# jgrss/cultionet

Measured on AMD Instinct MI355X. Metric: train_chips_per_sec, higher is better.
Workload: dtype f32

## Files before the change

### cultionet_amd/csrc/cn_conv.hip

```cpp
#include "cn_common.h"
#include "cn_conv_geom.h"
#include "cn_profile.h"

#include <cstdlib>

#define KC 8

static int cn_reduce_slices(const CnConvGeom& g, hipStream_t stream);

template <int TN, int TM>
__device__ __forceinline__ void cn_igemm_epilogue(const CnConvGeom& g, const f32x16 (&acc)[TN][TM],
                                                  const bool (&pix_ok)[TM], const int (&out_off)[TM], int co_base,
                                                  int half, int grp, int split, int b,
                                                  const float* __restrict__ bias, float* __restrict__ y) {
  const int HWout = g.Hout * g.Wout;
  const bool sliced = g.slice_stride != 0;
  float* yb = sliced ? g.part + (long)(grp * g.splits + split) * g.slice_stride + (long)b * g.Cout * HWout
                     : y + (long)b * g.ybs;
  const bool first = split == 0;
#pragma unroll
  for (int tn = 0; tn < TN; ++tn) {
#pragma unroll
    for (int r = 0; r < 16; ++r) {
      const int co = co_base + tn * 32 + (r & 3) + 8 * (r >> 2) + 4 * half;
      if (co < g.Cout) {
        const float bv = (bias != nullptr && first) ? bias[co] : 0.f;
#pragma unroll
        for (int tm = 0; tm < TM; ++tm) {
          if (pix_ok[tm]) {
            float* dst = yb + (long)co * HWout + out_off[tm];
            const float v = acc[tn][tm][r] + bv;
            if (sliced) {
              *dst = acc[tn][tm][r];
            } else if (g.atomic_out) {
              atomicAdd(dst, v);
            } else if (g.accumulate) {
              *dst += v;
            } else {
              *dst = v;
            }
          }
        }
      }
    }
  }
}

template <int WAVES_N, int TN, int NI_T>
__global__ __launch_bounds__(256) void cn_conv_igemm_kernel(const CnConvGeom g) {
  constexpr int WAVES_M = 4 / WAVES_N;
  constexpr int MT = WAVES_M * 64;
  constexpr int NT = WAVES_N * TN * 32;
  constexpr int WI = (CN_MAX_TAPS * KC * (NT / 4) + 255) / 256;
  extern __shared__ __attribute__((aligned(16))) float smem[];
  float* in_lds = smem;
  float* w_lds = smem + g.w_lds_off;
  int* tap_lds = reinterpret_cast<int*>(smem + g.tap_lds_off);

  const int tid = threadIdx.x, lane = tid & 63, wid = tid >> 6;
  const int half = lane >> 5, l31 = lane & 31;
  const int wm = wid / WAVES_N, wn = wid % WAVES_N;

  int bx, by, split;
  if (!cn_xcd_block(g.grid_x, g.grid_y, g.grid_x * g.grid_y * g.splits, bx, by, split)) return;
  int ci_ = 0;
  if (g.interleave) {
    ci_ = bx % g.ncls;
  } else {
#pragma unroll 1
    for (int c = 1; c < g.ncls; ++c)
      if (bx >= g.cls[c].block_begin) ci_ = c;
  }
  const int grp = g.cls[ci_].grp;
  const float* __restrict__ x = g.gx[grp];
  const float* __restrict__ wp = g.gwp[grp];
  const float* __restrict__ bias = g.gbias[grp];
  float* __restrict__ y = g.gy[grp];
  const int Hg = g.cls[ci_].Hg, Wg = g.cls[ci_].Wg, ntaps = g.cls[ci_].ntaps;
  const int pitch = g.cls[ci_].pitch, plane = g.cls[ci_].plane;
  const int min_dy = g.cls[ci_].min_dy, min_dx = g.cls[ci_].min_dx;
  const int oy0 = g.cls[ci_].oy0, ox0 = g.cls[ci_].ox0;
  const int tiles_per_img = g.cls[ci_].tiles_per_img;
  const int tile = g.interleave ? bx / g.ncls : bx - g.cls[ci_].block_begin;
  const int b = tile / tiles_per_img;
  const int m0 = (tile - b * tiles_per_img) * MT;
  if (tid < ntaps) {
    tap_lds[tid] = (g.cls[ci_].dy[tid] - min_dy) * pitch + (g.cls[ci_].dx[tid] - min_dx);
    tap_lds[CN_MAX_TAPS + tid] = g.cls[ci_].wt[tid];
  }
  __syncthreads();
  const int n0 = by * NT;
  const int Mimg = Hg * Wg;
  const int gy0 = m0 / Wg;
  const int iy_base = gy0 * g.is + min_dy;
  const int HWin = g.Hin * g.Win;

  int goff[NI_T];
#pragma unroll
  for (int i = 0; i < NI_T; ++i) {
    const int e = tid + i * 256;
    if (e < plane) {
      const int r = e / pitch, c = e - r * pitch;
      const int iy = iy_base + r, ix = c + min_dx;
      goff[i] = (iy >= 0 && iy < g.Hin && ix >= 0 && ix < g.Win) ? iy * g.Win + ix : -1;
    } else {
      goff[i] = -2;
    }
  }

  int pix_lds[2], out_off[2];
  bool pix_ok[2];
#pragma unroll
  for (int tm = 0; tm < 2; ++tm) {
    const int p = m0 + wm * 64 + tm * 32 + l31;
    pix_ok[tm] = p < Mimg;
    const int pc = pix_ok[tm] ? p : Mimg - 1;
    const int gy = pc / Wg, gx = pc - gy * Wg;
    pix_lds[tm] = ((gy - gy0) * g.is) * pitch + gx * g.is + half * plane;
    out_off[tm] = (gy * g.os + oy0) * g.Wout + gx * g.os + ox0;
  }

  f32x16 acc[TN][2];
#pragma unroll
  for (int tn = 0; tn < TN; ++tn)
#pragma unroll
    for (int tm = 0; tm < 2; ++tm)
#pragma unroll
      for (int r = 0; r < 16; ++r) acc[tn][tm][r] = 0.f;

  const float* xb = x + (long)b * g.xbs;
  const int nw4 = ntaps * KC * (NT / 4);
  const int nchunks = (g.Cin + KC - 1) / KC;
  int ch = split * g.chunks_per_split;
  int ch_end = ch + g.chunks_per_split;
  if (ch_end > nchunks) ch_end = nchunks;

  if (ntaps > 0 && ch < ch_end) {
    float xin[KC][NI_T];
    f32x4 win[WI];
    constexpr unsigned CN_OOBD = 0x80000000u;
    const __amdgpu_buffer_rsrc_t xrs =
        __builtin_amdgcn_make_buffer_rsrc(const_cast<float*>(xb), 0, 0x7fffffff, 0x00020000);
    const __amdgpu_buffer_rsrc_t wrs =
        __builtin_amdgcn_make_buffer_rsrc(const_cast<float*>(wp), 0, 0x7fffffff, 0x00020000);
    unsigned xo[NI_T], wo[WI];
#pragma unroll
    for (int i = 0; i < NI_T; ++i) xo[i] = goff[i] >= 0 ? (unsigned)goff[i] * 4u : CN_OOBD;
#pragma unroll
    for (int j = 0; j < WI; ++j) {
      const int f = tid + j * 256;
      wo[j] = CN_OOBD;
      if (f < nw4) {
        const int row = f / (NT / 4), c4 = f - row * (NT / 4);
        const int t = row / KC, ci = row - t * KC;
        wo[j] = (unsigned)(((tap_lds[CN_MAX_TAPS + t] * g.Kpad + ci) * g.Npad + n0 + c4 * 4) * 4);
      }
    }
#define CN_PREFETCH(c0_)                                                                                   \
  {                                                                                                        \
    const int c0 = (c0_);                                                                                  \
    _Pragma("unroll") for (int ci = 0; ci < KC; ++ci) {                                                    \
      if ((c0 + ci) < g.Cin) {                                                           \
        const int so = (c0 + ci) * HWin * 4;                                                               \
        _Pragma("unroll") for (int i = 0; i < NI_T; ++i)                                                   \
            xin[ci][i] = __builtin_bit_cast(float, __builtin_amdgcn_raw_buffer_load_b32(xrs, xo[i], so, 0)); \
      } else {                                                                                             \
        _Pragma("unroll") for (int i = 0; i < NI_T; ++i) xin[ci][i] = 0.f;                                 \
      }                                                                                                    \
    }                                                                                                      \
    const int wso = c0 * g.Npad * 4;                                                                       \
    _Pragma("unroll") for (int j = 0; j < WI; ++j)                                                         \
        win[j] = __builtin_bit_cast(f32x4, __builtin_amdgcn_raw_buffer_load_b128(wrs, wo[j], wso, 0));     \
  }
    CN_PREFETCH(ch * KC);
    for (; ch < ch_end; ++ch) {
      __syncthreads();
#pragma unroll
      for (int ci = 0; ci < KC; ++ci)
#pragma unroll
        for (int i = 0; i < NI_T; ++i)
          if (goff[i] != -2) in_lds[ci * plane + tid + i * 256] = xin[ci][i];
#pragma unroll
      for (int j = 0; j < WI; ++j) {
        const int f = tid + j * 256;
        if (f < nw4) *reinterpret_cast<f32x4*>(w_lds + f * 4) = win[j];
      }
      __syncthreads();
      if (ch + 1 < ch_end) CN_PREFETCH((ch + 1) * KC);
      float opa[2][TN], opb[2][2];
#define CN_LOAD_OPS(bf_, t_, cp_, toff_)                                                                   \
  {                                                                                                        \
    const float* wrow = w_lds + ((t_) * KC + half) * NT + wn * (TN * 32) + l31;                            \
    _Pragma("unroll") for (int tn = 0; tn < TN; ++tn) opa[bf_][tn] = wrow[(2 * (cp_)) * NT + tn * 32];     \
    opb[bf_][0] = in_lds[pix_lds[0] + (2 * (cp_)) * plane + (toff_)];                                      \
    opb[bf_][1] = in_lds[pix_lds[1] + (2 * (cp_)) * plane + (toff_)];                                      \
  }
#define CN_MFMA(bf_)                                                                                       \
  _Pragma("unroll") for (int tn = 0; tn < TN; ++tn) _Pragma("unroll") for (int tm = 0; tm < 2; ++tm)       \
      acc[tn][tm] = __builtin_amdgcn_mfma_f32_32x32x2f32(opa[bf_][tn], opb[bf_][tm], acc[tn][tm], 0, 0, 0);
      int toff_cur = tap_lds[0];
      CN_LOAD_OPS(0, 0, 0, toff_cur);
#pragma unroll 1
      for (int t = 0; t < ntaps; ++t) {
        const int toff_nxt = (t + 1 < ntaps) ? tap_lds[t + 1] : 0;
        CN_LOAD_OPS(1, t, 1, toff_cur);
        CN_MFMA(0);
        CN_LOAD_OPS(0, t, 2, toff_cur);
        CN_MFMA(1);
        CN_LOAD_OPS(1, t, 3, toff_cur);
        CN_MFMA(0);
        if (t + 1 < ntaps) CN_LOAD_OPS(0, t + 1, 0, toff_nxt);
        CN_MFMA(1);
        toff_cur = toff_nxt;
      }
#undef CN_LOAD_OPS
#undef CN_MFMA
    }
#undef CN_PREFETCH
  }

  cn_igemm_epilogue<TN, 2>(g, acc, pix_ok, out_off, n0 + wn * (TN * 32), half, grp, split, b, bias, y);
}

template <int WAVES_N, int TN, int TM, int NV, int RP>
__global__ __launch_bounds__(256, (NV <= 1 ? 2 : 1)) void cn_conv_igemm_vec_kernel(const CnConvGeom g) {
  constexpr int WAVES_M = 4 / WAVES_N;
  constexpr int MT = WAVES_M * TM * 32;
  constexpr int NT = WAVES_N * TN * 32;
  constexpr int WI = (CN_MAX_TAPS * KC * (NT / 4) + 255) / 256;
  constexpr int VS = NV * 1024;
  constexpr bool PADR = RP == 1 || RP == 2;
  constexpr int ODD = RP == 3 ? 1 : 0;
  constexpr int VSS = VS + ODD;
  extern __shared__ __attribute__((aligned(16))) float smem[];
  float* in_lds = smem;
  float* w_lds = smem + g.w_lds_off;
  int* tap_lds = reinterpret_cast<int*>(smem + g.tap_lds_off);

  const int tid = threadIdx.x, lane = tid & 63, wid = tid >> 6;
  const int half = lane >> 5, l31 = lane & 31;
  const int wm = wid / WAVES_N, wn = wid % WAVES_N;

  int bx, by, split;
  if (!cn_xcd_block(g.grid_x, g.grid_y, g.grid_x * g.grid_y * g.splits, bx, by, split)) return;
  int ci_ = 0;
  if (g.interleave) {
    ci_ = bx % g.ncls;
  } else {
#pragma unroll 1
    for (int c = 1; c < g.ncls; ++c)
      if (bx >= g.cls[c].block_begin) ci_ = c;
  }
  const int grp = g.cls[ci_].grp;
  const float* __restrict__ x = g.gx[grp];
  const float* __restrict__ wp = g.gwp[grp];
  const float* __restrict__ bias = g.gbias[grp];
  float* __restrict__ y = g.gy[grp];
  const int Hg = g.cls[ci_].Hg, Wg = g.cls[ci_].Wg, ntaps = g.cls[ci_].ntaps;
  const int vplane = g.cls[ci_].vplane;
  const int min_dy = g.cls[ci_].min_dy, min_dx = g.cls[ci_].min_dx;
  const int oy0 = g.cls[ci_].oy0, ox0 = g.cls[ci_].ox0;
  const int tiles_per_img = g.cls[ci_].tiles_per_img;
  const int tile = g.interleave ? bx / g.ncls : bx - g.cls[ci_].block_begin;
  const int b = tile / tiles_per_img;
  const int m0 = (tile - b * tiles_per_img) * MT;
  const int Win = g.Win;
  const int pitch = PADR ? ((Win + 3) / 4 * 4 + 4) : Win;
  if (tid < ntaps) {
    tap_lds[tid] = PADR ? (g.cls[ci_].dy[tid] - min_dy) * pitch + g.cls[ci_].dx[tid]
                      : (g.cls[ci_].dy[tid] - min_dy) * Win + (g.cls[ci_].dx[tid] - min_dx);
    tap_lds[CN_MAX_TAPS + tid] = g.cls[ci_].wt[tid];
    tap_lds[2 * CN_MAX_TAPS + tid] = g.cls[ci_].dx[tid];
  }
  __syncthreads();
  const int n0 = by * NT;
  const int Mimg = Hg * Wg;
  const int gy0 = m0 / Wg;
  const int HWin = g.Hin * Win;
  const int start = PADR ? (gy0 * g.is + min_dy) * Win : (gy0 * g.is + min_dy) * Win + min_dx;
  const int f0 = (start >> 2) << 2;
  const int sh = start - f0;

  int goff[NV];
  int ldst[NV];
  int ldst2[NV];
#pragma unroll
  for (int i = 0; i < NV; ++i) {
    const int e4 = 4 * (tid + i * 256) - (PADR ? sh : 0);
    const int lim = PADR ? g.cls[ci_].rows * Win : vplane;
    ldst[i] = 0;
    ldst2[i] = 0;
    if (e4 + 3 >= 0 && e4 < lim) {
      const int fq = start + e4 - (PADR ? 0 : sh);
      goff[i] = (fq >= 0 && (ODD ? fq < HWin : fq + 3 < HWin)) ? fq : -1;
      if (RP == 1) {
        const int r = e4 / Win;
        ldst[i] = r * pitch + 4 + (e4 - r * Win);
      } else if (RP == 2) {
        const int ea = e4 < 0 ? e4 + 2 : e4, eb = e4 + 2;
        const int ra = ea / Win, rb = eb / Win;
        ldst[i] = e4 < 0 ? -1 : ra * pitch + 4 + (ea - ra * Win);
        ldst2[i] = eb < lim ? rb * pitch + 4 + (eb - rb * Win) : -1;
      } else {
        ldst[i] = e4;
      }
    } else {
      goff[i] = -2;
    }
  }
  if (PADR) {
    for (int e = tid; e < KC * VS; e += 256) in_lds[e] = 0.f;
  }

  int pix_lds[TM], out_off[TM];
  unsigned colmask[TM];
  bool pix_ok[TM];
#pragma unroll
  for (int tm = 0; tm < TM; ++tm) {
    const int p = m0 + wm * (TM * 32) + tm * 32 + l31;
    pix_ok[tm] = p < Mimg;
    const int pc = pix_ok[tm] ? p : Mimg - 1;
    const int gy = pc / Wg, gx = pc - gy * Wg;
    pix_lds[tm] = PADR ? ((gy - gy0) * g.is) * pitch + 4 + gx * g.is + half * VS
                     : ((gy - gy0) * g.is) * Win + gx * g.is + sh + half * VSS;
    out_off[tm] = (gy * g.os + oy0) * g.Wout + gx * g.os + ox0;
    unsigned m = 0;
    for (int t = 0; t < ntaps; ++t) {
      const int ix = gx * g.is + tap_lds[2 * CN_MAX_TAPS + t];
      if (ix >= 0 && ix < Win) m |= 1u << t;
    }
    colmask[tm] = m;
  }

  f32x16 acc[TN][TM];
#pragma unroll
  for (int tn = 0; tn < TN; ++tn)
#pragma unroll
    for (int tm = 0; tm < TM; ++tm)
#pragma unroll
      for (int r = 0; r < 16; ++r) acc[tn][tm][r] = 0.f;
  const float* xb = x + (long)b * g.xbs;
  const int nw4 = ntaps * KC * (NT / 4);
  const int nchunks = (g.Cin + KC - 1) / KC;
  int ch = split * g.chunks_per_split;
  int ch_end = ch + g.chunks_per_split;
  if (ch_end > nchunks) ch_end = nchunks;

  if (ntaps > 0 && ch < ch_end) {
    f32x4 xin[KC][NV];
    f32x4 win[WI];
    constexpr unsigned CN_OOB = 0x80000000u;
    const __amdgpu_buffer_rsrc_t xrs =
        __builtin_amdgcn_make_buffer_rsrc(const_cast<float*>(xb), 0, 0x7fffffff, 0x00020000);
    const __amdgpu_buffer_rsrc_t wrs =
        __builtin_amdgcn_make_buffer_rsrc(const_cast<float*>(wp), 0, 0x7fffffff, 0x00020000);
    unsigned xo[NV], wo[WI];
#pragma unroll
    for (int i = 0; i < NV; ++i) xo[i] = goff[i] >= 0 ? (unsigned)goff[i] * 4u : CN_OOB;
#pragma unroll
    for (int j = 0; j < WI; ++j) {
      const int f = tid + j * 256;
      wo[j] = CN_OOB;
      if (f < nw4) {
        const int row = f / (NT / 4), c4 = f - row * (NT / 4);
        const int t = row / KC, ci = row - t * KC;
        wo[j] = (unsigned)(((tap_lds[CN_MAX_TAPS + t] * g.Kpad + ci) * g.Npad + n0 + c4 * 4) * 4);
      }
    }
#define CN_PREFETCH_V(c0_)                                                                                 \
  {                                                                                                        \
    const int c0 = (c0_);                                                                                  \
    _Pragma("unroll") for (int ci = 0; ci < KC; ++ci) {                                                    \
      if ((c0 + ci) < g.Cin) {                                                           \
        const int so = ODD ? (((c0 + ci) * HWin) & ~3) * 4 : (c0 + ci) * HWin * 4;                                                               \
        _Pragma("unroll") for (int i = 0; i < NV; ++i)                                                     \
            xin[ci][i] = __builtin_bit_cast(f32x4, __builtin_amdgcn_raw_buffer_load_b128(xrs, xo[i], so, 0)); \
      } else {                                                                                             \
        _Pragma("unroll") for (int i = 0; i < NV; ++i) xin[ci][i] = f32x4{0.f, 0.f, 0.f, 0.f};             \
      }                                                                                                    \
    }                                                                                                      \
    const int wso = c0 * g.Npad * 4;                                                                       \
    _Pragma("unroll") for (int j = 0; j < WI; ++j)                                                         \
        win[j] = __builtin_bit_cast(f32x4, __builtin_amdgcn_raw_buffer_load_b128(wrs, wo[j], wso, 0));     \
  }
    CN_PREFETCH_V(ch * KC);
    for (; ch < ch_end; ++ch) {
      __syncthreads();
#pragma unroll
      for (int ci = 0; ci < KC; ++ci)
#pragma unroll
        for (int i = 0; i < NV; ++i)
          if (goff[i] != -2) {
            if (RP == 2) {
              if (ldst[i] >= 0) *reinterpret_cast<float2*>(in_lds + ci * VS + ldst[i]) = make_float2(xin[ci][i][0], xin[ci][i][1]);
              if (ldst2[i] >= 0) *reinterpret_cast<float2*>(in_lds + ci * VS + ldst2[i]) = make_float2(xin[ci][i][2], xin[ci][i][3]);
            } else if (ODD) {
              f32x4 v = xin[ci][i];
              const int dl = ci & 3;
              const bool first = dl > 0 && goff[i] == 0;
              const bool last = dl < 3 && goff[i] == HWin - 1;
#pragma unroll
              for (int j = 0; j < 4; ++j)
                if ((first && j < dl) || (last && j > dl)) v[j] = 0.f;
              *reinterpret_cast<f32x4*>(in_lds + ci * VS + (ci & ~3) + ldst[i]) = v;
            } else {
              *reinterpret_cast<f32x4*>(in_lds + ci * VS + ldst[i]) = xin[ci][i];
            }
          }
#pragma unroll
      for (int j = 0; j < WI; ++j) {
        const int f = tid + j * 256;
        if (f < nw4) *reinterpret_cast<f32x4*>(w_lds + f * 4) = win[j];
      }
      __syncthreads();
      if (ch + 1 < ch_end) CN_PREFETCH_V((ch + 1) * KC);
#pragma unroll 1
      for (int t = 0; t < ntaps; ++t) {
        const int toff = tap_lds[t];
        const float* wrow = w_lds + (t * KC + half) * NT + wn * (TN * 32) + l31;
        const float* brow[TM];
        int msk[TM];
#pragma unroll
        for (int tm = 0; tm < TM; ++tm) {
          brow[tm] = in_lds + pix_lds[tm] + toff;
          msk[tm] = PADR ? -1 : __builtin_amdgcn_sbfe((int)colmask[tm], t, 1);
        }
#pragma unroll
        for (int cp = 0; cp < KC / 2; ++cp) {
          float a[TN], bb[TM];
#pragma unroll
          for (int tn = 0; tn < TN; ++tn) a[tn] = wrow[(2 * cp) * NT + tn * 32];
#pragma unroll
          for (int tm = 0; tm < TM; ++tm)
            bb[tm] = PADR ? brow[tm][(2 * cp) * VS] : __int_as_float(__float_as_int(brow[tm][(2 * cp) * VSS]) & msk[tm]);
#pragma unroll
          for (int tn = 0; tn < TN; ++tn)
#pragma unroll
            for (int tm = 0; tm < TM; ++tm)
              acc[tn][tm] = __builtin_amdgcn_mfma_f32_32x32x2f32(a[tn], bb[tm], acc[tn][tm], 0, 0, 0);
        }
      }
    }
#undef CN_PREFETCH_V
  }

  cn_igemm_epilogue<TN, TM>(g, acc, pix_ok, out_off, n0 + wn * (TN * 32), half, grp, split, b, bias, y);
}

__global__ void cn_pack_weights_kernel(const float* __restrict__ w, float* __restrict__ wp, int T, int K,
                                       int N, int Kpad, int Npad, long sk, long sn, long st) {
  const long total = (long)T * Kpad * Npad;
  for (long i = blockIdx.x * (long)blockDim.x + threadIdx.x; i < total; i += (long)gridDim.x * blockDim.x) {
    const int n = (int)(i % Npad);
    const long r = i / Npad;
    const int k = (int)(r % Kpad);
    const int t = (int)(r / Kpad);
    wp[i] = (k < K && n < N) ? w[k * sk + n * sn + t * st] : 0.f;
  }
}

struct CnPackDesc {
  const float* w;
  float* wp;
  int T, K, N, Kpad, Npad;
  long sk, sn, st;
};

#define CN_PK_TS 32
#define CN_PK_PITCH (32 * CN_MAX_TAPS + 1)
__global__ __launch_bounds__(256) void cn_pack_weights_batched_kernel(const CnPackDesc* __restrict__ descs) {
  __shared__ float tile[CN_PK_TS * CN_PK_PITCH];
  const CnPackDesc d = descs[blockIdx.y];
  const bool n_slow = d.sn > d.sk;
  const long ss = n_slow ? d.sn : d.sk, sm = n_slow ? d.sk : d.sn;
  const int S = n_slow ? d.N : d.K, M = n_slow ? d.K : d.N;
  const int Spad = n_slow ? d.Npad : d.Kpad, Mpad = n_slow ? d.Kpad : d.Npad;
  if (d.T > CN_MAX_TAPS || d.st != 1 || sm != d.T) {
    const long total = (long)d.T * d.Kpad * d.Npad;
    for (long i = blockIdx.x * (long)blockDim.x + threadIdx.x; i < total; i += (long)gridDim.x * blockDim.x) {
      const int n = (int)(i % d.Npad);
      const long r = i / d.Npad;
      const int k = (int)(r % d.Kpad);
      const int t = (int)(r / d.Kpad);
      d.wp[i] = (k < d.K && n < d.N) ? d.w[k * d.sk + n * d.sn + t * d.st] : 0.f;
    }
    return;
  }
  const int T = d.T;
  const int ts = (Spad + CN_PK_TS - 1) / CN_PK_TS, tm = (Mpad + 31) / 32;
  const int run = 32 * T;
  for (int tl = blockIdx.x; tl < ts * tm; tl += gridDim.x) {
    const int s0 = (tl / tm) * CN_PK_TS, m0 = (tl % tm) * 32;
    __syncthreads();
    for (int s = threadIdx.x >> 6; s < CN_PK_TS; s += 4)
      for (int j = threadIdx.x & 63; j < run; j += 64) {
        const long mi = (long)m0 * T + j;
        tile[s * CN_PK_PITCH + j] = (s0 + s < S && mi < (long)M * T) ? d.w[(s0 + s) * ss + mi] : 0.f;
      }
    __syncthreads();
// ... 201 lines not shown
      if (splits != sp && !forced) continue;
      const double cost = cn_launch_cost(base * splits, cps, chunk_units, splits, out_elems);
      if (cost < best.cost * (i == best.cfg ? 1.0 : 0.98)) best = {i, splits, cps, cost};
    }
  }
  return best;
}


#include <mutex>
#include <unordered_map>
namespace {
struct CnWs { float* p; long n; };
std::mutex g_ws_mu;
std::unordered_map<void*, CnWs> g_ws_by_stream;
}

extern "C" int cn_conv_set_workspace(void* stream, float* ws, long ws_floats) {
  if (ws != nullptr && ((reinterpret_cast<uintptr_t>(ws) & 15) || ws_floats < 0)) return CN_ERR_ARG;
  std::lock_guard<std::mutex> lk(g_ws_mu);
  if (ws == nullptr) g_ws_by_stream.erase(stream);
  else g_ws_by_stream[stream] = {ws, ws_floats};
  return CN_OK;
}

static void cn_bind_ws(void* stream) {
  std::lock_guard<std::mutex> lk(g_ws_mu);
  auto it = g_ws_by_stream.find(stream);
  if (it == g_ws_by_stream.end()) { g_conv_ws = nullptr; g_conv_ws_floats = 0; }
  else { g_conv_ws = it->second.p; g_conv_ws_floats = it->second.n; }
}

struct CnReduceArgs {
  const float* part;
  long slice_stride;
  int nsum;
  int ngrp;
  float* y[CN_MAX_GROUPS];
  const float* bias[CN_MAX_GROUPS * CN_MAX_GROUPS];
  int nbias;
  long ybs;
  int B, Cout, HW, accumulate;
};

__global__ __launch_bounds__(256) void cn_conv_reduce_kernel(const CnReduceArgs a) {
  const long n = (long)a.Cout * a.HW;
  const int b = blockIdx.y, gi = blockIdx.z;
  const float* p0 = a.part + (long)gi * a.nsum * a.slice_stride + (long)b * n;
  float* yb = a.y[gi] + (long)b * a.ybs;
  for (long i = (blockIdx.x * 256L + threadIdx.x) * 4; i < n; i += (long)gridDim.x * 1024) {
    if (i + 3 < n && (n & 3) == 0 && (a.ybs & 3) == 0 && (reinterpret_cast<uintptr_t>(yb) & 15) == 0) {
      f32x4 s = *reinterpret_cast<const f32x4*>(p0 + i);
      for (int k = 1; k < a.nsum; ++k) s += *reinterpret_cast<const f32x4*>(p0 + (long)k * a.slice_stride + i);
#pragma unroll
      for (int e = 0; e < 4; ++e) {
        const int c = (int)((i + e) / a.HW);
        for (int j = 0; j < a.nbias; ++j)
          if (a.bias[gi * CN_MAX_GROUPS + j] != nullptr) s[e] += a.bias[gi * CN_MAX_GROUPS + j][c];
      }
      f32x4* d = reinterpret_cast<f32x4*>(yb + i);
      *d = a.accumulate ? *d + s : s;
    } else {
      for (long e = i; e < n && e < i + 4; ++e) {
        float s = p0[e];
        for (int k = 1; k < a.nsum; ++k) s += p0[(long)k * a.slice_stride + e];
        const int c = (int)(e / a.HW);
        for (int j = 0; j < a.nbias; ++j)
          if (a.bias[gi * CN_MAX_GROUPS + j] != nullptr) s += a.bias[gi * CN_MAX_GROUPS + j][c];
        yb[e] = a.accumulate ? yb[e] + s : s;
      }
    }
  }
}

static int cn_finish_split(CnConvGeom& g, const CnPlan& p, int splits, int cps, float* y, hipStream_t stream) {
  (void)y;
  const int nchunks = (g.Cin + KC - 1) / KC;
  g.chunks_per_split = cps > 0 ? cps : (nchunks > 0 ? nchunks : 1);
  if (p.max_taps == 0) g.chunks_per_split = nchunks > 0 ? nchunks : 1;
  g.splits = splits < 1 ? 1 : splits;
  g.atomic_out = g.splits > 1 || (g.G > 1 && g.shared_y);
  g.part = nullptr;
  g.slice_stride = 0;
  if (g.atomic_out) {
    const long stride = ((long)g.B * g.Cout * g.Hout * g.Wout + 3) / 4 * 4;
    if (g_conv_ws != nullptr && stride * g.G * g.splits <= g_conv_ws_floats) {
      g.part = g_conv_ws;
      g.slice_stride = stride;
      return CN_OK;
    }
  }
  if (g.atomic_out && !g.accumulate) {
    const int ny = g.shared_y ? 1 : g.G;
    for (int i = 0; i < ny; ++i)
      if (hipMemsetAsync(g.gy[i], 0, sizeof(float) * (size_t)g.B * g.Cout * g.Hout * g.Wout, stream) != hipSuccess)
        return CN_ERR_LAUNCH;
  }
  return CN_OK;
}

static int cn_reduce_slices(const CnConvGeom& g, hipStream_t stream) {
  if (g.slice_stride == 0) return CN_OK;
  CnReduceArgs a = {};
  a.part = g.part;
  a.slice_stride = g.slice_stride;
  a.ybs = g.ybs; a.B = g.B; a.Cout = g.Cout; a.HW = g.Hout * g.Wout; a.accumulate = g.accumulate;
  if (g.shared_y) {
    a.nsum = g.G * g.splits; a.ngrp = 1; a.y[0] = g.gy[0]; a.nbias = g.G;
    for (int j = 0; j < g.G; ++j) a.bias[j] = g.gbias[j];
  } else {
    a.nsum = g.splits; a.ngrp = g.G; a.nbias = 1;
    for (int i = 0; i < g.G; ++i) { a.y[i] = g.gy[i]; a.bias[i * CN_MAX_GROUPS] = g.gbias[i]; }
  }
  const long n = (long)g.Cout * a.HW;
  long bx = (n + 1023) / 1024;
  if (bx > 1024) bx = 1024;
  CN_LAUNCH(cn_conv_reduce_kernel, dim3((unsigned)bx, g.B, a.ngrp), dim3(256), 0, stream, a);
  return cn_check_launch();
}

template <int WAVES_N, int TN, int TM>
static int cn_launch_vec_cfg(const float* x, const float* wp, const float* bias, float* y, CnConvGeom& g, int splits,
                             int cps, hipStream_t stream) {
  constexpr int MT = (4 / WAVES_N) * TM * 32;
  const CnPlan p = cn_plan(g, MT);
  if (p.total_tiles <= 0) return CN_OK;
  const int rp = g.odd_planes ? 3
                 : (p.max_rplane <= 4096 && p.max_absdx <= 4) ? (g.Win % 4 == 0 ? 1 : (g.Win % 2 == 0 ? 2 : 0)) : 0;
  const int img = (rp == 1 || rp == 2) ? p.max_rplane : p.max_vplane;
  g.w_lds_off = KC * 1024 * (img <= 1024 ? 1 : (img <= 2048 ? 2 : 4)) + (rp == 3 ? 16 : 0);
  const int rc = cn_finish_split(g, p, splits, cps, y, stream);
  if (rc != CN_OK) return rc;
#define CN_GO(NV_, RP_) \
  return cn_launch_igemm_v<WAVES_N, TN, TM, NV_, RP_>(x, wp, bias, y, g, p.total_tiles, p.max_taps, splits, p.flops, stream)
  if (rp == 1) {
    if (img <= 1024) CN_GO(1, 1);
    if (img <= 2048) CN_GO(2, 1);
    CN_GO(4, 1);
  }
  if (rp == 2) {
    if (img <= 1024) CN_GO(1, 2);
    if (img <= 2048) CN_GO(2, 2);
    CN_GO(4, 2);
  }
  if (rp == 3) {
    if (img <= 1024) CN_GO(1, 3);
    if (img <= 2048) CN_GO(2, 3);
    CN_GO(4, 3);
  }
  if (img <= 1024) CN_GO(1, 0);
  if (img <= 2048) CN_GO(2, 0);
  CN_GO(4, 0);
#undef CN_GO
}

template <int WAVES_N, int TN>
static int cn_launch_dword_cfg(const float* x, const float* wp, const float* bias, float* y, CnConvGeom& g,
                               int splits, int cps, hipStream_t stream) {
  constexpr int MT = (4 / WAVES_N) * 64;
  const CnPlan p = cn_plan(g, MT);
  if (p.total_tiles <= 0) return CN_OK;
  if (p.max_plane > 12 * 256) return CN_ERR_LDS;
  g.w_lds_off = (KC * p.max_plane + 3) / 4 * 4;
  const int rc = cn_finish_split(g, p, splits, cps, y, stream);
  if (rc != CN_OK) return rc;
  if (p.max_plane <= 3 * 256)
// ... 252 lines not shown
    const long stride = ((long)g.B * g.Cout * g.Hout * g.Wout + 3) / 4 * 4;
    ws_cap = g_conv_ws_floats / (stride * (g.G > 0 ? g.G : 1));
  }
  hipEvent_t e0, e1;
  if (hipEventCreate(&e0) != hipSuccess || hipEventCreate(&e1) != hipSuccess) return model;
  CnChoice best = model;
  float best_ms = 1e30f;
  for (int i = 0; i < ncfg; ++i) {
    CnConvGeom gi = g;
    const CnPlan p = cn_plan(gi, mts[i]);
    if (p.total_tiles <= 0) continue;
    int max_splits = (allow_split && p.max_taps > 0 && nchunks >= 4) ? nchunks / 2 : 1;
    if (max_splits > 32) max_splits = 32;
    if (max_splits > ws_cap) max_splits = ws_cap < 1 ? 1 : (int)ws_cap;
    for (int sp : split_set) {
      if (sp > max_splits) break;
      const int cps = (nchunks + sp - 1) / sp;
      const int splits = (nchunks + cps - 1) / cps;
      if (splits != sp) continue;
      if ((long)p.total_tiles * ny * splits > 8192) continue;
      const CnChoice c = {i, splits, cps, 0.0};
      float ms = 0.f;
      bool ok = true;
      for (int rep = 0; rep < 2 && ok; ++rep) {
        CnConvGeom gg = g;
        ok = hipEventRecord(e0, stream) == hipSuccess && run(c, gg) == CN_OK &&
             hipEventRecord(e1, stream) == hipSuccess && hipEventSynchronize(e1) == hipSuccess &&
             hipEventElapsedTime(&ms, e0, e1) == hipSuccess;
      }
      if (ok && ms < best_ms) { best_ms = ms; best = c; }
    }
  }
  (void)hipEventDestroy(e0);
  (void)hipEventDestroy(e1);
  return best;
}

int cn_conv_igemm_launch(CnConvGeom& g, hipStream_t stream) {
  if (g.ncls < 1 || g.ncls > CN_MAX_CLASSES || g.B <= 0 || g.G < 1) return g.B <= 0 ? CN_OK : CN_ERR_ARG;
  g.splits = 1;
  const float* x = g.gx[0]; const float* wp = g.gwp[0]; const float* bias = g.gbias[0]; float* y = g.gy[0];
  g.Kpad = cn_conv_kpad(g.Cin);
  g.Npad = cn_conv_npad(g.Cout);
  const int nt = cn_pick_nt(g.Cout);
  const bool dense_out = g.ybs == (long)g.Cout * g.Hout * g.Wout;
  const bool ws_fits = g_conv_ws != nullptr &&
                       (((long)g.B * g.Cout * g.Hout * g.Wout + 3) / 4 * 4) * g.G * 32 <= g_conv_ws_floats;
  const bool allow_split = dense_out || g.accumulate || ws_fits;
  if (g.G > 1 && g.shared_y && !allow_split) return CN_ERR_ARG;
  const int hw4 = (int)(((long)g.Hin * g.Win) % 4);
  g.odd_planes = (hw4 == 1 && !(g.is > 1 && (long)g.Hin * g.Win > 4096)) ? 1 : 0;
  bool vec = (hw4 == 0 || g.odd_planes) && (g.xbs % 4 == 0);
  if (g.is > 1 && (long)g.Hin * g.Win > 4096) vec = false;
  if ((long)g.Cin * g.Hin * g.Win * 4 >= (1L << 31) || (long)CN_MAX_TAPS * cn_conv_kpad(g.Cin) * g.Npad * 4 >= (1L << 31))
    return CN_ERR_ARG;
  for (int i = 0; i < g.G; ++i) vec = vec && ((reinterpret_cast<uintptr_t>(g.gx[i]) & 15) == 0);
  if (vec) {
    CnConvGeom t = g;
    vec = cn_plan(t, 256).max_vplane <= 4 * 1024;
  }
  static const int mts128[3] = {128, 96, 160};
  static const int mts128d[1] = {128};
  static const int mts256[1] = {256};
  const int* mts = nt == 128 ? (vec ? mts128 : mts128d) : mts256;
  const int ncfg = (nt == 128 && vec) ? 3 : 1;
  auto run = [&](const CnChoice& c, CnConvGeom& gg) -> int {
    if (nt == 128) {
      if (vec) {
        switch (c.cfg) {
          case 1: return cn_launch_vec_cfg<4, 1, 3>(x, wp, bias, y, gg, c.splits, c.cps, stream);
          case 2: return cn_launch_vec_cfg<4, 1, 5>(x, wp, bias, y, gg, c.splits, c.cps, stream);
          default: return cn_launch_vec_cfg<2, 2, 2>(x, wp, bias, y, gg, c.splits, c.cps, stream);
        }
      }
      return cn_launch_dword_cfg<2, 2>(x, wp, bias, y, gg, c.splits, c.cps, stream);
    }
    int rc;
    if (nt == 64) {
      if (vec) return cn_launch_vec_cfg<1, 2, 2>(x, wp, bias, y, gg, c.splits, c.cps, stream);
      rc = cn_launch_dword_cfg<1, 2>(x, wp, bias, y, gg, c.splits, c.cps, stream);
    } else {
      if (vec) return cn_launch_vec_cfg<1, 1, 2>(x, wp, bias, y, gg, c.splits, c.cps, stream);
      rc = cn_launch_dword_cfg<1, 1>(x, wp, bias, y, gg, c.splits, c.cps, stream);
    }
    if (rc == CN_ERR_LDS) {
      CnConvGeom g2 = gg;
      rc = cn_launch_dword_cfg<2, 2>(x, wp, bias, y, g2, c.splits, c.cps, stream);
    }
    return rc;
  };
  CnChoice c = cn_choose(g, mts, ncfg, nt, allow_split);
  if (g_autotune) {
    std::lock_guard<std::mutex> lk(g_tune_mu);
    const uint64_t key = cn_tune_key(g, vec, nt, allow_split);
    auto it = g_tuned.find(key);
    if (it != g_tuned.end()) {
      c = it->second;
    } else if (!g.accumulate && !cn_prof_on()) {
      c = cn_autotune(g, mts, ncfg, nt, allow_split, c, run, stream);
      g_tuned.emplace(key, c);
    }
  }
  return run(c, g);
}

static int cn_set_groups(CnConvGeom& g, int G, const float* const* xs, const float* const* wps,
                         const float* const* biases, float* const* ys) {
// ... 231 lines not shown
```

Measured before the change: 404.7.

## Issue first prefetch early, buffer-store epilogue, trim LDS zeroing and reduce bias work

Several changes are bundled here. The first chunk's global prefetch now issues before the pixel tables and accumulators are set up, to hide load latency when the N tile is at least 64. The epilogue switches to raw buffer stores with out-of-bounds masking, and the padded-row path zeroes only the gap columns in LDS instead of the whole buffer. The slice-reduce kernel skips bias work when there is none and hoists the per-channel bias lookup. Compile-gated diagnostic switches (no MFMA, no store, no tables) are also added, and the early prefetch keeps more registers live across setup, which may lower occupancy.

```diff
diff --git a/cultionet_amd/csrc/cn_conv.hip b/cultionet_amd/csrc/cn_conv.hip
--- a/cultionet_amd/csrc/cn_conv.hip
+++ b/cultionet_amd/csrc/cn_conv.hip
@@ -5,6 +5,19 @@
 #include <cstdlib>
 
 #define KC 8
+
+#define CN_DIAG_NO_MFMA 1
+#define CN_DIAG_NO_STORE 2
+#define CN_DIAG_NO_TABLES 4
+#ifdef CN_CONVDIAG
+__constant__ int cn_diag_bits;
+extern "C" int cn_conv_diag_mode(int bits) {
+  return hipMemcpyToSymbol(HIP_SYMBOL(cn_diag_bits), &bits, sizeof(int)) == hipSuccess ? CN_OK : CN_ERR_LAUNCH;
+}
+#define CN_DIAG(bit_) ((cn_diag_bits & (bit_)) != 0)
+#else
+#define CN_DIAG(bit_) false
+#endif
 
 static int cn_reduce_slices(const CnConvGeom& g, hipStream_t stream);
 
@@ -18,32 +31,54 @@
   float* yb = sliced ? g.part + (long)(grp * g.splits + split) * g.slice_stride + (long)b * g.Cout * HWout
                      : y + (long)b * g.ybs;
   const bool first = split == 0;
-#pragma unroll
-  for (int tn = 0; tn < TN; ++tn) {
-#pragma unroll
-    for (int r = 0; r < 16; ++r) {
-      const int co = co_base + tn * 32 + (r & 3) + 8 * (r >> 2) + 4 * half;
-      if (co < g.Cout) {
-        const float bv = (bias != nullptr && first) ? bias[co] : 0.f;
-#pragma unroll
-        for (int tm = 0; tm < TM; ++tm) {
-          if (pix_ok[tm]) {
-            float* dst = yb + (long)co * HWout + out_off[tm];
-            const float v = acc[tn][tm][r] + bv;
-            if (sliced) {
-              *dst = acc[tn][tm][r];
-            } else if (g.atomic_out) {
-              atomicAdd(dst, v);
-            } else if (g.accumulate) {
-              *dst += v;
-            } else {
-              *dst = v;
-            }
-          }
+  if (!sliced && g.atomic_out) {
+#pragma unroll
+    for (int tn = 0; tn < TN; ++tn) {
+#pragma unroll
+      for (int r = 0; r < 16; ++r) {
+        const int co = co_base + tn * 32 + (r & 3) + 8 * (r >> 2) + 4 * half;
+        if (co < g.Cout) {
+          const float bv = (bias != nullptr && first) ? bias[co] : 0.f;
+#pragma unroll
+          for (int tm = 0; tm < TM; ++tm)
+            if (pix_ok[tm]) atomicAdd(yb + (long)co * HWout + out_off[tm], acc[tn][tm][r] + bv);
         }
       }
     }
-  }
+    return;
+  }
+  constexpr unsigned CN_OOBS = 0x80000000u;
+  const __amdgpu_buffer_rsrc_t yrs = __builtin_amdgcn_make_buffer_rsrc(yb, 0, 0x7fffffff, 0x00020000);
+  const int co0 = co_base + 4 * half;
+  const int nco = g.Cout - co0;
+  unsigned po[TM];
+#pragma unroll
+  for (int tm = 0; tm < TM; ++tm) po[tm] = pix_ok[tm] ? (unsigned)(co0 * HWout + out_off[tm]) * 4u : CN_OOBS;
+  const bool add_bias = bias != nullptr && first && !sliced;
+  const int mode = sliced ? 0 : (g.accumulate ? 1 : 2);
+#define CN_EPI_ROWS(BODY_)                                                                                 \
+  _Pragma("unroll") for (int tn = 0; tn < TN; ++tn) _Pragma("unroll") for (int r = 0; r < 16; ++r) {       \
+    const int cu = tn * 32 + (r & 3) + 8 * (r >> 2);                                                       \
+    const bool cok = cu < nco;                                                                             \
+    const float bv = (add_bias && cok) ? bias[co0 + cu] : 0.f;                                             \
+    const int so = cu * HWout * 4;                                                                         \
+    _Pragma("unroll") for (int tm = 0; tm < TM; ++tm) {                                                    \
+      const unsigned vo = cok ? po[tm] : CN_OOBS;                                                          \
+      const float a = acc[tn][tm][r];                                                                      \
+      BODY_                                                                                                \
+    }                                                                                                      \
+  }
+#define CN_EPI_ST(v_) __builtin_amdgcn_raw_buffer_store_b32(__builtin_bit_cast(unsigned, (float)(v_)), yrs, vo, so, 0)
+  if (mode == 0) {
+    CN_EPI_ROWS(CN_EPI_ST(a);)
+  } else if (mode == 1) {
+    CN_EPI_ROWS(const float old = __builtin_bit_cast(float, __builtin_amdgcn_raw_buffer_load_b32(yrs, vo, so, 0));
+                CN_EPI_ST(old + (a + bv));)
+  } else {
+    CN_EPI_ROWS(CN_EPI_ST(a + bv);)
+  }
+#undef CN_EPI_ST
+#undef CN_EPI_ROWS
 }
 
 template <int WAVES_N, int TN, int NI_T>
@@ -52,6 +87,7 @@
   constexpr int MT = WAVES_M * 64;
   constexpr int NT = WAVES_N * TN * 32;
   constexpr int WI = (CN_MAX_TAPS * KC * (NT / 4) + 255) / 256;
+  constexpr bool EARLY = NT >= 64;
   extern __shared__ __attribute__((aligned(16))) float smem[];
   float* in_lds = smem;
   float* w_lds = smem + g.w_lds_off;
@@ -99,7 +135,9 @@
 #pragma unroll
   for (int i = 0; i < NI_T; ++i) {
     const int e = tid + i * 256;
-    if (e < plane) {
+    if (CN_DIAG(CN_DIAG_NO_TABLES)) {
+      goff[i] = e < plane ? (e < HWin ? e : -1) : -2;
+    } else if (e < plane) {
       const int r = e / pitch, c = e - r * pitch;
       const int iy = iy_base + r, ix = c + min_dx;
       goff[i] = (iy >= 0 && iy < g.Hin && ix >= 0 && ix < g.Win) ? iy * g.Win + ix : -1;
@@ -107,26 +145,6 @@
       goff[i] = -2;
     }
   }
-
-  int pix_lds[2], out_off[2];
-  bool pix_ok[2];
-#pragma unroll
-  for (int tm = 0; tm < 2; ++tm) {
-    const int p = m0 + wm * 64 + tm * 32 + l31;
-    pix_ok[tm] = p < Mimg;
-    const int pc = pix_ok[tm] ? p : Mimg - 1;
-    const int gy = pc / Wg, gx = pc - gy * Wg;
-    pix_lds[tm] = ((gy - gy0) * g.is) * pitch + gx * g.is + half * plane;
-    out_off[tm] = (gy * g.os + oy0) * g.Wout + gx * g.os + ox0;
-  }
-
-  f32x16 acc[TN][2];
-#pragma unroll
-  for (int tn = 0; tn < TN; ++tn)
-#pragma unroll
-    for (int tm = 0; tm < 2; ++tm)
-#pragma unroll
-      for (int r = 0; r < 16; ++r) acc[tn][tm][r] = 0.f;
 
   const float* xb = x + (long)b * g.xbs;
   const int nw4 = ntaps * KC * (NT / 4);
@@ -134,28 +152,27 @@
   int ch = split * g.chunks_per_split;
   int ch_end = ch + g.chunks_per_split;
   if (ch_end > nchunks) ch_end = nchunks;
-
-  if (ntaps > 0 && ch < ch_end) {
-    float xin[KC][NI_T];
-    f32x4 win[WI];
-    constexpr unsigned CN_OOBD = 0x80000000u;
-    const __amdgpu_buffer_rsrc_t xrs =
-        __builtin_amdgcn_make_buffer_rsrc(const_cast<float*>(xb), 0, 0x7fffffff, 0x00020000);
-    const __amdgpu_buffer_rsrc_t wrs =
-        __builtin_amdgcn_make_buffer_rsrc(const_cast<float*>(wp), 0, 0x7fffffff, 0x00020000);
-    unsigned xo[NI_T], wo[WI];
-#pragma unroll
-    for (int i = 0; i < NI_T; ++i) xo[i] = goff[i] >= 0 ? (unsigned)goff[i] * 4u : CN_OOBD;
-#pragma unroll
-    for (int j = 0; j < WI; ++j) {
-      const int f = tid + j * 256;
-      wo[j] = CN_OOBD;
-      if (f < nw4) {
-        const int row = f / (NT / 4), c4 = f - row * (NT / 4);
-        const int t = row / KC, ci = row - t * KC;
-        wo[j] = (unsigned)(((tap_lds[CN_MAX_TAPS + t] * g.Kpad + ci) * g.Npad + n0 + c4 * 4) * 4);
-      }
-    }
+  const bool work = ntaps > 0 && ch < ch_end;
+  float xin[KC][NI_T];
+  f32x4 win[WI];
+  constexpr unsigned CN_OOBD = 0x80000000u;
+  const __amdgpu_buffer_rsrc_t xrs =
+      __builtin_amdgcn_make_buffer_rsrc(const_cast<float*>(xb), 0, 0x7fffffff, 0x00020000);
+  const __amdgpu_buffer_rsrc_t wrs =
+      __builtin_amdgcn_make_buffer_rsrc(const_cast<float*>(wp), 0, 0x7fffffff, 0x00020000);
+  unsigned xo[NI_T], wo[WI];
+#pragma unroll
+  for (int i = 0; i < NI_T; ++i) xo[i] = goff[i] >= 0 ? (unsigned)goff[i] * 4u : CN_OOBD;
+#pragma unroll
+  for (int j = 0; j < WI; ++j) {
+    const int f = tid + j * 256;
+    wo[j] = CN_OOBD;
+    if (f < nw4) {
+      const int row = f / (NT / 4), c4 = f - row * (NT / 4);
+      const int t = row / KC, ci = row - t * KC;
+      wo[j] = (unsigned)(((tap_lds[CN_MAX_TAPS + t] * g.Kpad + ci) * g.Npad + n0 + c4 * 4) * 4);
+    }
+  }
 #define CN_PREFETCH(c0_)                                                                                   \
   {                                                                                                        \
     const int c0 = (c0_);                                                                                  \
@@ -172,7 +189,35 @@
     _Pragma("unroll") for (int j = 0; j < WI; ++j)                                                         \
         win[j] = __builtin_bit_cast(f32x4, __builtin_amdgcn_raw_buffer_load_b128(wrs, wo[j], wso, 0));     \
   }
-    CN_PREFETCH(ch * KC);
+  if (EARLY && work) CN_PREFETCH(ch * KC);
+
+  int pix_lds[2], out_off[2];
+  bool pix_ok[2];
+#pragma unroll
+  for (int tm = 0; tm < 2; ++tm) {
+    const int p = m0 + wm * 64 + tm * 32 + l31;
+    pix_ok[tm] = p < Mimg;
+    if (CN_DIAG(CN_DIAG_NO_TABLES)) {
+      pix_lds[tm] = l31 + half * plane;
+      out_off[tm] = p < g.Hout * g.Wout ? p : 0;
+      continue;
+    }
+    const int pc = pix_ok[tm] ? p : Mimg - 1;
+    const int gy = pc / Wg, gx = pc - gy * Wg;
+    pix_lds[tm] = ((gy - gy0) * g.is) * pitch + gx * g.is + half * plane;
+    out_off[tm] = (gy * g.os + oy0) * g.Wout + gx * g.os + ox0;
+  }
+
+  f32x16 acc[TN][2];
+#pragma unroll
+  for (int tn = 0; tn < TN; ++tn)
+#pragma unroll
+    for (int tm = 0; tm < 2; ++tm)
+#pragma unroll
+      for (int r = 0; r < 16; ++r) acc[tn][tm][r] = 0.f;
+
+  if (work) {
+    if (!EARLY) CN_PREFETCH(ch * KC);
     for (; ch < ch_end; ++ch) {
       __syncthreads();
 #pragma unroll
@@ -186,6 +231,7 @@
         if (f < nw4) *reinterpret_cast<f32x4*>(w_lds + f * 4) = win[j];
       }
       __syncthreads();
+      if (CN_DIAG(CN_DIAG_NO_MFMA)) break;
       if (ch + 1 < ch_end) CN_PREFETCH((ch + 1) * KC);
       float opa[2][TN], opb[2][2];
 #define CN_LOAD_OPS(bf_, t_, cp_, toff_)                                                                   \
@@ -219,7 +265,8 @@
 #undef CN_PREFETCH
   }
 
-  cn_igemm_epilogue<TN, 2>(g, acc, pix_ok, out_off, n0 + wn * (TN * 32), half, grp, split, b, bias, y);
+  if (!CN_DIAG(CN_DIAG_NO_STORE))
+    cn_igemm_epilogue<TN, 2>(g, acc, pix_ok, out_off, n0 + wn * (TN * 32), half, grp, split, b, bias, y);
 }
 
 template <int WAVES_N, int TN, int TM, int NV, int RP>
@@ -228,6 +275,7 @@
   constexpr int MT = WAVES_M * TM * 32;
   constexpr int NT = WAVES_N * TN * 32;
   constexpr int WI = (CN_MAX_TAPS * KC * (NT / 4) + 255) / 256;
+  constexpr bool EARLY = NT >= 64;
   constexpr int VS = NV * 1024;
   constexpr bool PADR = RP == 1 || RP == 2;
   constexpr int ODD = RP == 3 ? 1 : 0;
@@ -290,7 +338,12 @@
     const int lim = PADR ? g.cls[ci_].rows * Win : vplane;
     ldst[i] = 0;
     ldst2[i] = 0;
-    if (e4 + 3 >= 0 && e4 < lim) {
+    if (CN_DIAG(CN_DIAG_NO_TABLES)) {
+      const int q = 4 * (tid + i * 256);
+      goff[i] = (q + 3 < HWin && q + 16 <= VS) ? q : -2;
+      ldst[i] = q + 4;
+      ldst2[i] = q + 6;
+    } else if (e4 + 3 >= 0 && e4 < lim) {
       const int fq = start + e4 - (PADR ? 0 : sh);
       goff[i] = (fq >= 0 && (ODD ? fq < HWin : fq + 3 < HWin)) ? fq : -1;
       if (RP == 1) {
@@ -308,8 +361,64 @@
       goff[i] = -2;
     }
   }
-  if (PADR) {
-    for (int e = tid; e < KC * VS; e += 256) in_lds[e] = 0.f;
+  const float* xb = x + (long)b * g.xbs;
+  const int nw4 = ntaps * KC * (NT / 4);
+  const int nchunks = (g.Cin + KC - 1) / KC;
+  int ch = split * g.chunks_per_split;
+  int ch_end = ch + g.chunks_per_split;
+  if (ch_end > nchunks) ch_end = nchunks;
+  const bool work = ntaps > 0 && ch < ch_end;
+  f32x4 xin[KC][NV];
+  f32x4 win[WI];
+  constexpr unsigned CN_OOB = 0x80000000u;
+  const __amdgpu_buffer_rsrc_t xrs =
+      __builtin_amdgcn_make_buffer_rsrc(const_cast<float*>(xb), 0, 0x7fffffff, 0x00020000);
+  const __amdgpu_buffer_rsrc_t wrs =
+      __builtin_amdgcn_make_buffer_rsrc(const_cast<float*>(wp), 0, 0x7fffffff, 0x00020000);
+  unsigned xo[NV], wo[WI];
+#pragma unroll
+  for (int i = 0; i < NV; ++i) xo[i] = goff[i] >= 0 ? (unsigned)goff[i] * 4u : CN_OOB;
+#pragma unroll
+  for (int j = 0; j < WI; ++j) {
+    const int f = tid + j * 256;
+    wo[j] = CN_OOB;
+    if (f < nw4) {
+      const int row = f / (NT / 4), c4 = f - row * (NT / 4);
+      const int t = row / KC, ci = row - t * KC;
+      wo[j] = (unsigned)(((tap_lds[CN_MAX_TAPS + t] * g.Kpad + ci) * g.Npad + n0 + c4 * 4) * 4);
+    }
+  }
+#define CN_PREFETCH_V(c0_)                                                                                 \
+  {                                                                                                        \
+    const int c0 = (c0_);                                                                                  \
+    _Pragma("unroll") for (int ci = 0; ci < KC; ++ci) {                                                    \
+      if ((c0 + ci) < g.Cin) {                                                           \
+        const int so = ODD ? (((c0 + ci) * HWin) & ~3) * 4 : (c0 + ci) * HWin * 4;                         \
+        _Pragma("unroll") for (int i = 0; i < NV; ++i)                                                     \
+            xin[ci][i] = __builtin_bit_cast(f32x4, __builtin_amdgcn_raw_buffer_load_b128(xrs, xo[i], so, 0)); \
+      } else {                                                                                             \
+        _Pragma("unroll") for (int i = 0; i < NV; ++i) xin[ci][i] = f32x4{0.f, 0.f, 0.f, 0.f};             \
+      }                                                                                                    \
+    }                                                                                                      \
+    const int wso = c0 * g.Npad * 4;                                                                       \
+    _Pragma("unroll") for (int j = 0; j < WI; ++j)                                                         \
+        win[j] = __builtin_bit_cast(f32x4, __builtin_amdgcn_raw_buffer_load_b128(wrs, wo[j], wso, 0));     \
+  }
+  if (EARLY && work) CN_PREFETCH_V(ch * KC);
+
+  if (PADR && !CN_DIAG(CN_DIAG_NO_TABLES)) {
+    const int ngap = (g.cls[ci_].rows + 1) * KC;
+    for (int idx = tid; idx < ngap; idx += 256) {
+      const int r = idx / KC, ci = idx - r * KC;
+      float* gp = in_lds + ci * VS + (r == 0 ? 0 : (r - 1) * pitch + 4 + Win);
+      if (RP == 1) {
+        *reinterpret_cast<f32x4*>(gp) = f32x4{0.f, 0.f, 0.f, 0.f};
+      } else {
+        *reinterpret_cast<float2*>(gp) = make_float2(0.f, 0.f);
+        *reinterpret_cast<float2*>(gp + 2) = make_float2(0.f, 0.f);
+        if (r > 0) *reinterpret_cast<float2*>(gp + 4) = make_float2(0.f, 0.f);
+      }
+    }
   }
 
   int pix_lds[TM], out_off[TM];
@@ -319,6 +428,12 @@
   for (int tm = 0; tm < TM; ++tm) {
     const int p = m0 + wm * (TM * 32) + tm * 32 + l31;
     pix_ok[tm] = p < Mimg;
+    if (CN_DIAG(CN_DIAG_NO_TABLES)) {
+      pix_lds[tm] = 4 + l31 + half * VSS;
+      out_off[tm] = p < g.Hout * g.Wout ? p : 0;
+      colmask[tm] = ~0u;
+      continue;
+    }
     const int pc = pix_ok[tm] ? p : Mimg - 1;
     const int gy = pc / Wg, gx = pc - gy * Wg;
     pix_lds[tm] = PADR ? ((gy - gy0) * g.is) * pitch + 4 + gx * g.is + half * VS
@@ -339,51 +454,9 @@
     for (int tm = 0; tm < TM; ++tm)
 #pragma unroll
       for (int r = 0; r < 16; ++r) acc[tn][tm][r] = 0.f;
-  const float* xb = x + (long)b * g.xbs;
-  const int nw4 = ntaps * KC * (NT / 4);
-  const int nchunks = (g.Cin + KC - 1) / KC;
-  int ch = split * g.chunks_per_split;
-  int ch_end = ch + g.chunks_per_split;
-  if (ch_end > nchunks) ch_end = nchunks;
-
-  if (ntaps > 0 && ch < ch_end) {
-    f32x4 xin[KC][NV];
-    f32x4 win[WI];
-    constexpr unsigned CN_OOB = 0x80000000u;
-    const __amdgpu_buffer_rsrc_t xrs =
-        __builtin_amdgcn_make_buffer_rsrc(const_cast<float*>(xb), 0, 0x7fffffff, 0x00020000);
-    const __amdgpu_buffer_rsrc_t wrs =
-        __builtin_amdgcn_make_buffer_rsrc(const_cast<float*>(wp), 0, 0x7fffffff, 0x00020000);
-    unsigned xo[NV], wo[WI];
-#pragma unroll
-    for (int i = 0; i < NV; ++i) xo[i] = goff[i] >= 0 ? (unsigned)goff[i] * 4u : CN_OOB;
-#pragma unroll
-    for (int j = 0; j < WI; ++j) {
-      const int f = tid + j * 256;
-      wo[j] = CN_OOB;
-      if (f < nw4) {
-        const int row = f / (NT / 4), c4 = f - row * (NT / 4);
-        const int t = row / KC, ci = row - t * KC;
-        wo[j] = (unsigned)(((tap_lds[CN_MAX_TAPS + t] * g.Kpad + ci) * g.Npad + n0 + c4 * 4) * 4);
-      }
-    }
-#define CN_PREFETCH_V(c0_)                                                                                 \
-  {                                                                                                        \
-    const int c0 = (c0_);                                                                                  \
-    _Pragma("unroll") for (int ci = 0; ci < KC; ++ci) {                                                    \
-      if ((c0 + ci) < g.Cin) {                                                           \
-        const int so = ODD ? (((c0 + ci) * HWin) & ~3) * 4 : (c0 + ci) * HWin * 4;                                                               \
-        _Pragma("unroll") for (int i = 0; i < NV; ++i)                                                     \
-            xin[ci][i] = __builtin_bit_cast(f32x4, __builtin_amdgcn_raw_buffer_load_b128(xrs, xo[i], so, 0)); \
-      } else {                                                                                             \
-        _Pragma("unroll") for (int i = 0; i < NV; ++i) xin[ci][i] = f32x4{0.f, 0.f, 0.f, 0.f};             \
-      }                                                                                                    \
-    }                                                                                                      \
-    const int wso = c0 * g.Npad * 4;                                                                       \
-    _Pragma("unroll") for (int j = 0; j < WI; ++j)                                                         \
-        win[j] = __builtin_bit_cast(f32x4, __builtin_amdgcn_raw_buffer_load_b128(wrs, wo[j], wso, 0));     \
-  }
-    CN_PREFETCH_V(ch * KC);
+
+  if (work) {
+    if (!EARLY) CN_PREFETCH_V(ch * KC);
     for (; ch < ch_end; ++ch) {
       __syncthreads();
 #pragma unroll
@@ -413,6 +486,7 @@
         if (f < nw4) *reinterpret_cast<f32x4*>(w_lds + f * 4) = win[j];
       }
       __syncthreads();
+      if (CN_DIAG(CN_DIAG_NO_MFMA)) break;
       if (ch + 1 < ch_end) CN_PREFETCH_V((ch + 1) * KC);
 #pragma unroll 1
       for (int t = 0; t < ntaps; ++t) {
@@ -444,7 +518,8 @@
 #undef CN_PREFETCH_V
   }
 
-  cn_igemm_epilogue<TN, TM>(g, acc, pix_ok, out_off, n0 + wn * (TN * 32), half, grp, split, b, bias, y);
+  if (!CN_DIAG(CN_DIAG_NO_STORE))
+    cn_igemm_epilogue<TN, TM>(g, acc, pix_ok, out_off, n0 + wn * (TN * 32), half, grp, split, b, bias, y);
 }
 
 __global__ void cn_pack_weights_kernel(const float* __restrict__ w, float* __restrict__ wp, int T, int K,
@@ -752,11 +827,23 @@
     if (i + 3 < n && (n & 3) == 0 && (a.ybs & 3) == 0 && (reinterpret_cast<uintptr_t>(yb) & 15) == 0) {
       f32x4 s = *reinterpret_cast<const f32x4*>(p0 + i);
       for (int k = 1; k < a.nsum; ++k) s += *reinterpret_cast<const f32x4*>(p0 + (long)k * a.slice_stride + i);
-#pragma unroll
-      for (int e = 0; e < 4; ++e) {
-        const int c = (int)((i + e) / a.HW);
-        for (int j = 0; j < a.nbias; ++j)
-          if (a.bias[gi * CN_MAX_GROUPS + j] != nullptr) s[e] += a.bias[gi * CN_MAX_GROUPS + j][c];
+      if (a.nbias > 0) {
+        if ((a.HW & 3) == 0) {
+          const int c = (int)(i / a.HW);
+          for (int j = 0; j < a.nbias; ++j)
+            if (a.bias[gi * CN_MAX_GROUPS + j] != nullptr) {
+              const float bv = a.bias[gi * CN_MAX_GROUPS + j][c];
+#pragma unroll
+              for (int e = 0; e < 4; ++e) s[e] += bv;
+            }
+        } else {
+#pragma unroll
+          for (int e = 0; e < 4; ++e) {
+            const int c = (int)((i + e) / a.HW);
+            for (int j = 0; j < a.nbias; ++j)
+              if (a.bias[gi * CN_MAX_GROUPS + j] != nullptr) s[e] += a.bias[gi * CN_MAX_GROUPS + j][c];
+          }
+        }
       }
       f32x4* d = reinterpret_cast<f32x4*>(yb + i);
       *d = a.accumulate ? *d + s : s;
@@ -764,9 +851,11 @@
       for (long e = i; e < n && e < i + 4; ++e) {
         float s = p0[e];
         for (int k = 1; k < a.nsum; ++k) s += p0[(long)k * a.slice_stride + e];
-        const int c = (int)(e / a.HW);
-        for (int j = 0; j < a.nbias; ++j)
-          if (a.bias[gi * CN_MAX_GROUPS + j] != nullptr) s += a.bias[gi * CN_MAX_GROUPS + j][c];
+        if (a.nbias > 0) {
+          const int c = (int)(e / a.HW);
+          for (int j = 0; j < a.nbias; ++j)
+            if (a.bias[gi * CN_MAX_GROUPS + j] != nullptr) s += a.bias[gi * CN_MAX_GROUPS + j][c];
+        }
         yb[e] = a.accumulate ? yb[e] + s : s;
       }
     }
@@ -812,6 +901,7 @@
     a.nsum = g.splits; a.ngrp = g.G; a.nbias = 1;
     for (int i = 0; i < g.G; ++i) { a.y[i] = g.gy[i]; a.bias[i * CN_MAX_GROUPS] = g.gbias[i]; }
   }
+  if (!g.has_bias) a.nbias = 0;
   const long n = (long)g.Cout * a.HW;
   long bx = (n + 1023) / 1024;
   if (bx > 1024) bx = 1024;
@@ -1170,7 +1260,8 @@
   g.odd_planes = (hw4 == 1 && !(g.is > 1 && (long)g.Hin * g.Win > 4096)) ? 1 : 0;
   bool vec = (hw4 == 0 || g.odd_planes) && (g.xbs % 4 == 0);
   if (g.is > 1 && (long)g.Hin * g.Win > 4096) vec = false;
-  if ((long)g.Cin * g.Hin * g.Win * 4 >= (1L << 31) || (long)CN_MAX_TAPS * cn_conv_kpad(g.Cin) * g.Npad * 4 >= (1L << 31))
+  if ((long)g.Cin * g.Hin * g.Win * 4 >= (1L << 31) || (long)CN_MAX_TAPS * cn_conv_kpad(g.Cin) * g.Npad * 4 >= (1L << 31) ||
+      (long)g.Cout * g.Hout * g.Wout * 4 >= (1L << 31))
     return CN_ERR_ARG;
   for (int i = 0; i < g.G; ++i) vec = vec && ((reinterpret_cast<uintptr_t>(g.gx[i]) & 15) == 0);
   if (vec) {
```

Result: no change. 405.0, median of 2 (+0.1%).
